# JakobHavtorn/benchmarking-lvms

Hardware: AMD Instinct MI355X
Metric: audio frames/sec training (VRNN, 16 kHz mu-law) (higher is better)
Workload: dtype f32

## Files before the change

### benchmarking-lvms_amd/csrc/pchain.h

```cpp
#pragma once
#include <algorithm>
#include <cstdlib>

#include "common.h"
#include "decode_tiles.h"

namespace blvm {
namespace pchain {

constexpr unsigned SENTINEL = 0xFFFFFFFFu;
constexpr unsigned SPIN_LIMIT = 1u << 22;

typedef unsigned u32x4 __attribute__((ext_vector_type(4)));
typedef __amdgpu_buffer_rsrc_t rsrc_t;
constexpr int AUX_SC1 = 16;
#ifndef PCHAIN_POLL_AUX
#define PCHAIN_POLL_AUX AUX_SC1
#endif
#ifndef PCHAIN_STORE_AUX
#define PCHAIN_STORE_AUX AUX_SC1
#endif
__device__ __forceinline__ rsrc_t make_rsrc(const void* base) {
  const unsigned long long u = reinterpret_cast<unsigned long long>(base);
  const unsigned lo = (unsigned)__builtin_amdgcn_readfirstlane((int)(unsigned)u), hi = (unsigned)__builtin_amdgcn_readfirstlane((int)(unsigned)(u >> 32));
// ... 1198 lines not shown
inline SeqLink rev_link(const float* W, const float* gate, float* orm, float* o16, long t0, long sB, int ld, long x16) {
  return SeqLink{W, gate ? gate + t0 * sB : nullptr, orm ? orm + t0 * sB : nullptr, -sB, ld, o16 ? o16 + t0 * x16 : nullptr};
}
inline int range_for(int tiles, int avail) { return std::max(8, std::min(avail & ~7, (tiles + 7) & ~7)); }

}

hipError_t pchain_fill_sentinel(void* p, size_t bytes, hipStream_t stream);
inline int pchain_ctl(pchain::Ctl& c) { return pchain_ctl(&c.dev, &c.host, &c.epoch); }
int pchain_prepare(pchain::Builder& bld, const char* who);
int pchain_run(const pchain::Program& prog, hipStream_t stream);
inline int pchain_launch(pchain::Builder& bld, const char* who, hipStream_t stream) {
  BLVM_TRY(pchain_prepare(bld, who));
  return pchain_run(bld.p, stream);
}
int vrnn_launch(pchain::Builder& bld, bool forward, const char* who, hipStream_t stream);
int pchain_rows_to_t16(const float* src, int ld, int B, int K, float* dst, hipStream_t stream, int n16 = 0, int k_src = 0);
struct StackPad {
  int S, Sp, N, Np;
  bool padded() const { return Sp != S; }
  size_t stage_in(int H) const { return padded() ? (size_t)H * Sp : 0; }
  size_t stage_dec(int H) const { return padded() ? (size_t)Np * H : 0; }
  size_t stage_bias() const { return padded() ? (size_t)Np : 0; }
};
inline StackPad stack_pad(int S, int F) {
  const int Sp = (S + 15) / 16 * 16, N = S * F;
  return StackPad{S, Sp, N, Sp != S ? (N + 15) / 16 * 16 : N};
}
inline int pad_copy(float* dst, int rows_p, int cols_p, const float* src, int rows, int cols, hipStream_t s) {
  BLVM_HIP(hipMemsetAsync(dst, 0, sizeof(float) * (size_t)rows_p * cols_p, s));
  BLVM_HIP(hipMemcpy2DAsync(dst, sizeof(float) * cols_p, src, sizeof(float) * cols, sizeof(float) * cols, rows, hipMemcpyDeviceToDevice, s));
// ... 21 lines not shown
```

### benchmarking-lvms_amd/csrc/vrnn.hip

```cpp
#include <vector>
#include <stdlib.h>

#include <algorithm>

#include "common.h"
#include "pchain.h"
#include "vrnn_static.h"

namespace blvm {
namespace {

#include "stages.h"


template <int NW>
__global__ __launch_bounds__(NW * 64) void gru_stage_kernel(const float* decin_t, const float* Wih, const float* xg,
                                                            const float* gh, int B, int H, int R, float* decin_next,
                                                            float* rg, float* ug, float* ng) {
  __shared__ float red[3 * NW * 256];
  const int r0 = blockIdx.y * 16, c0 = blockIdx.x * 16, wave = threadIdx.x >> 6;
  const int ldd = H + R;
  const int t = threadIdx.x & 255;
  const int row = r0 + (t >> 4), col = c0 + (t & 15);
  const bool own = threadIdx.x < 256 && row < B;
// ... 282 lines not shown
    BLVM_TRY(t16_pack_rows(w->post_w[l], H, H, H, rs.Wq[l], s));
  }
  BLVM_TRY(t16_pack_rows(w->prior_hw, H, 2 * Z, H, rs.Wph, s));
  BLVM_TRY(t16_pack_rows(w->post_hw, H, 2 * Z, H, rs.Wqh, s));
  BLVM_TRY(t16_pack_rows(w->phi_w[0], Z, H, Z, rs.Wf[0], s));
  for (int l = 1; l < 4; ++l) BLVM_TRY(t16_pack_rows(w->phi_w[l], H, H, H, rs.Wf[l], s));
  BLVM_TRY(t16_pack_rows(w->gru_wih + X, X + H, 3 * R, H, rs.Wih, s));
  BLVM_TRY(t16_pack_rows(w->gru_whh, R, 3 * R, R, rs.Whh, s));
  if (fold) {
    BLVM_TRY(t16_pack_rows(dec->w[0], H + R, H, H + R, rs.Wd[0], s));
    BLVM_TRY(t16_pack_rows(dec->w[1], H, H, H, rs.Wd[1], s));
    if (fold == 3) BLVM_TRY(t16_pack_rows(dec->w[2], H, SF, H, rs.Wd[2], s));
  }
  BLVM_TRY(pack_scope.flush());

  BLVM_HIP(copy_or_zero_2d(decin + H, sizeof(float) * ldd, h0, sizeof(float) * R, B, s));
  BLVM_HIP(hipMemset2DAsync(decin + n * ldd, sizeof(float) * ldd, 0, sizeof(float) * H, B, s));

  const int rt = (B + 15) / 16;
  if (vrnn_persistent(B) && device_cus() >= 32) {
    using namespace pchain;
    const int ctH = H / 16, ctZ = Z / 16, ctR = R / 16, cus = device_cus() & ~7;
    const long sH = (long)B * H, sZ = (long)B * Z, sR = (long)B * R, s3R = 3 * sR, sD = (long)B * ldd;
    const long xH = (long)rt * 16 * H, xZ = (long)rt * 16 * Z, xR = (long)rt * 16 * R;
    const bool groups = vrnn_row_groups(B);
    const int RTG = groups ? vrnn_rt(B) : 1;
    const int tl = (rt + RTG - 1) / RTG;
    const bool shared = vrnn_shared_deal(groups, tl);
    const VrnnFwdDeal dl = vrnn_fwd_deal(ctH, ctZ, ctR, tl, cus, shared, dec_ct(fold, SF));
    Builder bld;
    bld.begin(pchain_optype(B), Tp, B, groups ? 8 : 4, false, dl.g);
// ... 49 lines not shown
      o = Operands();
      o.p[LIN_A] = {rs.PHI16, xH}; o.p[LIN_W] = rs.Wd[0]; o.i[LIN_I_W_WIDTH] = ldw; o.p[LIN_ADD] = {rs.Y1P, sH}; o.ld[LIN_LD_ADD] = H;
      o.p[LIN_ORM] = {dec->y[0], sH}; o.ld[LD_OUT] = H; o.p[LIN_O16] = {rs.Y116, xH}; o.n16[N16_OUT] = ctH; o.f[LIN_F_SLOPE] = dec_slope;
      add_desc(bld, K_LIN, dl.dec[1].ct, dl.dec[1].wg0, dl.dec[1].nwg, H, DF_ADD_POLLED | DF_RELU | DF_GENTLE | canary, 0, Tp, o);
      o = Operands();
      o.p[LIN_A] = {rs.Y116, xH}; o.p[LIN_W] = rs.Wd[1]; o.p[LIN_BIAS] = dec->b[1]; o.p[LIN_ORM] = {dec->y[1], sH}; o.ld[LD_OUT] = H;
      o.p[LIN_O16] = {rs.Y216, xH}; o.n16[N16_OUT] = ctH; o.f[LIN_F_SLOPE] = dec_slope;
      add_desc(bld, K_LIN, dl.dec[2].ct, dl.dec[2].wg0, dl.dec[2].nwg, H, DF_RELU | DF_GENTLE | canary, 0, Tp, o);
      if (fold == 3) {
        o = Operands();
        o.p[LIN_A] = {rs.Y216, xH}; o.p[LIN_W] = rs.Wd[2]; o.p[LIN_BIAS] = dec->b[2]; o.p[LIN_ORM] = {dec->y[2], sF}; o.ld[LD_OUT] = SF;
        o.f[LIN_F_SLOPE] = dec_slope;
        add_desc(bld, K_LIN, dl.dec[3].ct, dl.dec[3].wg0, dl.dec[3].nwg, H, DF_RELU | DF_GENTLE | canary, 0, Tp, o);
      }
    }
    BLVM_HIP(pchain_fill_sentinel(rs.H16, rs.x16_bytes, s));
    BLVM_HIP(pchain_fill_sentinel(rs.GHb, sizeof(float) * n * 3 * R, s));
    BLVM_HIP(pchain_fill_sentinel(decin, sizeof(float) * n * ldd, s));
    BLVM_HIP(copy_or_zero_2d(decin + H, sizeof(float) * ldd, h0, sizeof(float) * R, B, s));
    BLVM_TRY(pchain_rows_to_t16(h0, R, B, R, rs.H16, s));
    BLVM_TRY(vrnn_launch(bld, true, "vrnn_fwd", s));
    if (fold) { ++g_dec_folded; if (folded) *folded = fold; }
    return BLVM_OK;
  }
  for (int t = 0; t < Tp; ++t) {
    const size_t oH = (size_t)t * B * H, oZ = (size_t)t * B * Z, oR = (size_t)t * B * R, o3R = (size_t)t * B * 3 * R;
    const float* dec_t = decin + (size_t)t * B * ldd;
    float* dec_n = decin + (size_t)(t + 1) * B * ldd;
    const float* hprev = dec_t + H;
    LinLaunch a;
    a.B = B;
    a.nseg = 3;
    a.seg[0] = seg(hprev, ldd, rs.Wp[0], R, w->prior_b[0], nullptr, 0, nullptr, 0, rs.P[0] + oH, H, H, R, 1);
    a.seg[1] = seg(hprev, ldd, rs.Wq[0], R, nullptr, rs.XQ + oH, H, nullptr, 0, rs.Q[0] + oH, H, H, R, 1);
    a.seg[2] = seg(hprev, ldd, rs.Whh, R, w->gru_bhh, nullptr, 0, nullptr, 0, rs.GHb + o3R, 3 * R, 3 * R, R, 0);
    launch_lin(a, s);
// ... 202 lines not shown
    {
      Operands z;
      z.p[DZ_D16] = last(ws.DPHI16[0], xH); z.p[DZ_WT] = ws.fT[0]; z.p[DZ_MU_Q] = last(mu_q, sZ); z.p[DZ_SD_Q] = last(sd_q, sZ); z.p[DZ_MU_P] = last(mu_p, sZ);
      z.p[DZ_SD_P] = last(sd_p, sZ); z.p[DZ_EPS] = last(eps, sZ); z.p[DZ_RAW_Q] = last(rs.RAWQ, sZ); z.p[DZ_RAW_P] = last(rs.RAWP, sZ); z.p[DZ_X_SL] = x_sl;
      z.p[DZ_C_RAW] = c_raw; z.p[DZ_C_FN] = c_fn; z.p[DZ_DQH] = last(ws.DQH, s2Z); z.p[DZ_DQH16] = last(ws.DQH16, x2Z); z.p[DZ_DPH] = last(ws.DPH, s2Z);
      z.p[DZ_DPH16] = last(ws.DPH16, x2Z); z.ld[LD_OUT] = 2 * Z; z.n16[N16_OUT] = 2 * ctZ; z.i[DZ_I_Z] = Z; z.i[DZ_I_RESIDUAL] = residual_posterior;
      z.i[DZ_I_STRIDE] = stride; z.i[DZ_I_T0] = T - 1; z.f[DZ_F_FN_FLOOR] = fn_floor; z.f[DZ_F_BETA] = beta; z.f[DZ_F_SD_EPS] = sd_eps;
      add_desc(bld, K_DZ, ctZ, dl.dz.wg0, dl.dz.nwg, H, 0, 0, T, z);
    }
    {
      const SeqLink lp[3] = {blink(ws.phT, rs.P[2], ws.DP[2], ws.DP16[2]), blink(ws.pT[2], rs.P[1], ws.DP[1], ws.DP16[1]), blink(ws.pT[1], rs.P[0], ws.DP[0], ws.DP16[0])};
      const SeqLink lq[3] = {blink(ws.qhT, rs.Q[2], ws.DQ[2], ws.DQ16[2]), blink(ws.qT[2], rs.Q[1], ws.DQ[1], ws.DQ16[1]), blink(ws.qT[1], rs.Q[0], ws.DQ[0], ws.DQ16[0])};
      add_linseq(bld, ctH, dl.prior.wg0, dl.prior.nwg, H, false, true, 0, T, last(ws.DPH16, x2Z), 3, lp, -sH, -xH, ctH, 0.f, H, 2 * Z);
      add_linseq(bld, ctH, dl.post.wg0, dl.post.nwg, H, false, true, 0, T, last(ws.DQH16, x2Z), 3, lq, -sH, -xH, ctH, 0.f, H, 2 * Z);
    }
    BLVM_HIP(pchain_fill_sentinel(ws.GA, ws.x16_bytes, s));
    BLVM_TRY(vrnn_launch(bld, false, "vrnn_bwd", s));
    if (split3) {
      const size_t n4 = n * H / 4;
      hipLaunchKernelGGL(add3_kernel, dim3((unsigned)std::min<size_t>((n4 + 255) / 256, 2048)), dim3(256), 0, s, reinterpret_cast<float4*>(ws.DPHI[3]),
                         reinterpret_cast<const float4*>(ws.DPHI3b), reinterpret_cast<const float4*>(ws.DPHI3c), n4);
    }
    return batched();
  }

  launch_dh(-1, Tp - 1);
  for (int t = Tp - 1; t >= 0; --t) {
    const size_t oH = (size_t)t * B * H, oZ = (size_t)t * B * Z, o3R = (size_t)t * B * 3 * R, o2Z = (size_t)t * B * 2 * Z;
    const float* dec_t = decin + (size_t)t * B * ldd;
    const float* ddec_t = d_decin + (size_t)t * B * ldd;
    LinLaunch a;
    a.B = B;
// ... 45 lines not shown
```

### benchmarking-lvms_amd/csrc/vrnn_static.h

```cpp
#pragma once
#include <algorithm>
#include <initializer_list>

#include "pchain.h"

namespace blvm {
namespace pchain {

struct LinkRange {
  int ct, wg0, nwg;
};
constexpr int kMaxTiles = 8;
struct VrnnFwdDeal {
  int def_n, half, g, spare;
  LinkRange hproj, prior, post, head, phi, gru, dec[4];
};
inline VrnnFwdDeal vrnn_fwd_deal(int ctH, int ctZ, int ctR, int tl, int cus, bool shared, int ctD = 0) {
  VrnnFwdDeal d;
  d.def_n = shared ? 0 : range_for(3 * ctR * tl, std::min(cus / 4, 64));
  d.half = range_for(ctH * tl, (cus - d.def_n) / 2);
  d.g = 2 * d.half;
  const int wide = shared ? d.half : d.g;
  d.hproj = shared ? LinkRange{3 * ctR, d.half, d.half} : LinkRange{3 * ctR, d.g, d.def_n};
  d.prior = LinkRange{ctH, 0, d.half};
// ... 68 lines not shown
    if (!kept) return false;
  }
  return true;
}
inline int place_for(int want, int fallback, const Program& p, int prior, int post, int grid) {
  if (want == kPlaceLocal) return place_local_applies(p, prior, post, grid) ? kPlaceLocal : (fallback == kPlacePlain ? kPlacePlain : kPlaceProgram);
  return want == kPlacePlain ? kPlacePlain : kPlaceProgram;
}
inline bool place_xcd(int place, const Program& p) { return place == kPlaceProgram && p.xcd != 0; }
inline int grid_of(const Program& p) {
  int g = 0;
  for (int i = 0; i < p.ndesc; ++i) g = std::max(g, p.d[i].wg0 + p.d[i].nwg);
  return g;
}

}
}
```

### benchmarking-lvms_amd/csrc/vrnn_static.hip

```cpp
#include <algorithm>
#include <mutex>

#include "common.h"
#include "pchain.h"
#include "vrnn_static.h"

namespace blvm {
namespace {
using namespace pchain;

struct SPtr {
  float* base;
  int stride;
  __device__ __forceinline__ float* at(int s) const { return base + (long)s * stride; }
};

__device__ __forceinline__ int placed_wg(int place) { return place == kPlaceLocal ? place_wg((int)blockIdx.x) : (int)blockIdx.x; }
__device__ __forceinline__ int tile_lanes(int w, int wg0, int nwg, int rt, int ct, bool xcd) {
  TileIter it(w, wg0, nwg, rt, ct, xcd);
  const int lane = threadIdx.x & 63;
  it.j += lane * it.step;
  return (lane < kMaxTiles && it.valid()) ? (it.r0() | (it.c() << 16)) : -1;
}
__device__ __forceinline__ int tile_count(int lanes) { return __popcll(__ballot(lanes >= 0)); }
// ... 281 lines not shown
  if (nt == 0 || s < d.s_begin || s >= d.s_end) return;
  wk.at(d, s, false);
  GrubIn g;
  g.D0 = q.D0.at(s); g.D1 = q.D1.at(s); g.W0 = q.W0; g.W1 = q.W1; g.g_in = q.g_in.at(s); g.g_add = q.g_add.at(s); g.ld_gadd = q.ld1;
  g.rg = q.rg.at(s); g.ug = q.ug.at(s); g.ng = q.ng.at(s); g.gh = q.gh.at(s); g.hprev = q.hprev.at(s); g.dd = q.dd.at(s); g.ldh = q.ld0;
  g.dgi = Out{q.dgi.at(s), q.ld3, false, q.dgi16.at(s), q.n16};
  g.dgh = Out{q.dgh.at(s), q.ld3, false, q.dgh16.at(s), q.n16};
  g.ga = q.ga.at(s); g.g_out = const_cast<float*>(q.g_out);
  g.has_gemm = s >= q.first_gemm; g.has_gates = s < q.end_gates; g.has_gin = s >= q.first_gin;
  const int trc = __builtin_amdgcn_readlane(tiles, 0);
  ANAT(anat_arm(wk.pl);)
  tile_grub<NW, OP_F32>(g, kH, q.R, trc & 0xffff, (trc >> 16) * 16, wk.B, wk.red(), wk.pl, ws, PC());
  ANAT(anat_note(wk.anat, 4 * d.idx, wk.pl);)
}

template <class A>
__device__ __forceinline__ const A& kargs() {
  typedef const __attribute__((address_space(4))) char kchar;
  kchar* p = (kchar*)__builtin_amdgcn_kernarg_segment_ptr();
  asm volatile("" : "+s"(p));
  return *(const A*)p;
}

struct FwdArgs {
  LinArgs hproj;
  SeqArgs run[2];
  HeadArgs head;
  SeqArgs phi;
  GruArgs gru;
  LinArgs dec[4];
  Deal deal[kFwdDecDesc];
  int ndec;
  int B, s0, S, xcd, place;
  Ctl ctl;
  ANAT(unsigned long long* prof;)
};
constexpr int kFwdProducts = 4, kBwdProducts = 2;

template <int NW, int HALF>
__device__ __forceinline__ void fwd_half(const FwdArgs& a, int w, int rt, bool xcd, Walk& wk) {
  const int t1 = tile_lanes(w, a.deal[1 + HALF].wg0, a.deal[1 + HALF].nwg, rt, a.deal[1 + HALF].ct, xcd), n1 = tile_count(t1);
  const int t3 = tile_lanes(w, a.deal[3].wg0, a.deal[3].nwg, rt, a.deal[3].ct, xcd), n3 = tile_count(t3);
  const int t4 = tile_lanes(w, a.deal[4].wg0, a.deal[4].nwg, rt, a.deal[4].ct, xcd), n4 = tile_count(t4);
  const int t5 = tile_lanes(w, a.deal[5].wg0, a.deal[5].nwg, rt, a.deal[5].ct, xcd), n5 = tile_count(t5);
  RunRes<3, kR, kH> run;
  Res<kH, 4> head;
  RunRes<4, kH, kH> phi;
  Res<kH, 3> gru;
  load_run<NW>(run, kargs<FwdArgs>().run[HALF], t1, n1);
  load_head<NW>(head, kargs<FwdArgs>().head, t3, n3);
  load_run<NW>(phi, kargs<FwdArgs>().phi, t4, n4);
  load_gru<NW>(gru, kargs<FwdArgs>().gru, t5, n5);
  for (int s = a.s0; s < a.S; ++s) {
    visit_run<NW, 3, kR, kH, false, Paced>(kargs<FwdArgs>().run[HALF], kargs<FwdArgs>().deal[1 + HALF], s, t1, n1, wk, run);
    visit_head<NW, Paced>(kargs<FwdArgs>().head, kargs<FwdArgs>().deal[3], s, t3, n3, wk, head);
    visit_run<NW, 4, kH, kH, false, Paced>(kargs<FwdArgs>().phi, kargs<FwdArgs>().deal[4], s, t4, n4, wk, phi);
    if constexpr (HALF == 0) visit_gru<NW, Paced>(kargs<FwdArgs>().gru, kargs<FwdArgs>().deal[5], s, t5, n5, wk, gru);
    else visit_gru<NW>(kargs<FwdArgs>().gru, kargs<FwdArgs>().deal[5], s, t5, n5, wk, gru);
  }
  ANAT(anat_end(wk.anat, kargs<FwdArgs>().prof, HALF, w == kargs<FwdArgs>().deal[1 + HALF].wg0);)
}

constexpr int kDecFlags = DF_RELU | DF_GENTLE | DF_CANARY;
template <int NW>
__device__ __forceinline__ void fwd_dec(const FwdArgs& a, int w, int rt, bool xcd, Walk& wk) {
  const int t6 = tile_lanes(w, a.deal[6].wg0, a.deal[6].nwg, rt, a.deal[6].ct, xcd), n6 = tile_count(t6);
  const int t7 = tile_lanes(w, a.deal[7].wg0, a.deal[7].nwg, rt, a.deal[7].ct, xcd), n7 = tile_count(t7);
  const int t8 = tile_lanes(w, a.deal[8].wg0, a.deal[8].nwg, rt, a.deal[8].ct, xcd), n8 = tile_count(t8);
  const int t9 = tile_lanes(w, a.deal[9].wg0, a.deal[9].nwg, rt, a.deal[9].ct, xcd), n9 = tile_count(t9);
  if ((n6 | n7 | n8 | n9) == 0) return;
  Res<kR> w1h;
  Res<kH> w1p, w2;
  load_lin<NW, kR>(w1h, kargs<FwdArgs>().dec[0].W, kargs<FwdArgs>().dec[0].w_width, t6, n6);
  load_lin<NW, kH>(w1p, kargs<FwdArgs>().dec[1].W, kargs<FwdArgs>().dec[1].w_width, t7, n7);
  load_lin<NW, kH>(w2, kargs<FwdArgs>().dec[2].W, kH, t8, n8);
  for (int s = a.s0; s < a.S; ++s) {
    visit_lin<NW, kR, DF_RM_SC1 | DF_GENTLE | DF_CANARY>(kargs<FwdArgs>().dec[0], kargs<FwdArgs>().deal[6], s, t6, n6, wk, w1h);
// ... 9 lines not shown
  const int w = placed_wg(a.place), rt = (a.B + 15) / 16;
  const bool xcd = a.place == kPlaceProgram && a.xcd != 0;
  Walk wk{lds_red, lds_red + kFwdProducts * NW * 256, 0, a.B, Poll{a.ctl, 0u, false, 1}};
  ANAT(__shared__ unsigned anat[kAnatSlots * 8]; anat_begin(anat); wk.anat = anat;)
  if (a.ndec != 0 && w >= a.deal[6].wg0) {
    fwd_dec<NW>(a, w, rt, xcd, wk);
    return;
  }
  if (w >= a.deal[0].wg0) {
    const int t0 = tile_lanes(w, a.deal[0].wg0, a.deal[0].nwg, rt, a.deal[0].ct, xcd), n0 = tile_count(t0);
    if (n0 == 0) return;
    for (int s = a.s0; s < a.S; ++s) visit_lin<NW, kR, DF_RM_SC1 | DF_GENTLE | DF_CANARY>(kargs<FwdArgs>().hproj, kargs<FwdArgs>().deal[0], s, t0, n0, wk, WMem());
    return;
  }
  if (w < a.deal[2].wg0) fwd_half<NW, 0>(a, w, rt, xcd, wk);
  else fwd_half<NW, 1>(a, w, rt, xcd, wk);
}

struct BwdArgs {
  GrubArgs grub;
  LinArgs part[3], gb, sum;
  SeqArgs phi;
  DzArgs dz;
  SeqArgs run[2];
  Deal deal[10];
  int B, s0, S, xcd, place;
  Ctl ctl;
  ANAT(unsigned long long* prof;)
};

template <int NW, int HALF>
__device__ __forceinline__ void bwd_half(const BwdArgs& a, int w, int rt, bool xcd, Walk& wk) {
  const int t0 = tile_lanes(w, a.deal[0].wg0, a.deal[0].nwg, rt, a.deal[0].ct, xcd), n0 = tile_count(t0);
  const int t1 = tile_lanes(w, a.deal[1 + HALF].wg0, a.deal[1 + HALF].nwg, rt, a.deal[1 + HALF].ct, xcd), n1 = tile_count(t1);
  const int t5 = tile_lanes(w, a.deal[5].wg0, a.deal[5].nwg, rt, a.deal[5].ct, xcd), n5 = tile_count(t5);
  const int t6 = tile_lanes(w, a.deal[6].wg0, a.deal[6].nwg, rt, a.deal[6].ct, xcd), n6 = tile_count(t6);
  const int t7 = tile_lanes(w, a.deal[7].wg0, a.deal[7].nwg, rt, a.deal[7].ct, xcd), n7 = tile_count(t7);
  const int t8 = tile_lanes(w, a.deal[8 + HALF].wg0, a.deal[8 + HALF].nwg, rt, a.deal[8 + HALF].ct, xcd), n8 = tile_count(t8);
  Res<kH, 2> grub;
  Res<kR> part;
  Res<kH> sum, dz;
  RunRes<2, kH, kH> phi;
// ... 16 lines not shown
  ANAT(anat_end(wk.anat, kargs<BwdArgs>().prof, 2 + HALF, w == kargs<BwdArgs>().deal[1 + HALF].wg0);)
}

template <int NW>
__global__ __launch_bounds__(NW * 64, 1) void vrnn_static_bwd_kernel(BwdArgs a) {
  extern __shared__ __attribute__((aligned(16))) float lds_red[];
  const int w = placed_wg(a.place), rt = (a.B + 15) / 16;
  const bool xcd = a.place == kPlaceProgram && a.xcd != 0;
  Walk wk{lds_red, lds_red + kBwdProducts * NW * 256, 0, a.B, Poll{a.ctl, 0u, false, 1}};
  ANAT(__shared__ unsigned anat[kAnatSlots * 8]; anat_begin(anat); wk.anat = anat;)
  if (w >= a.deal[3].wg0) {
    const int t = tile_lanes(w, a.deal[3].wg0, a.deal[3].nwg, rt, a.deal[3].ct, xcd), n = tile_count(t);
    if (n == 0) return;
    Res<kR> part;
    load_lin<NW, kR>(part, kargs<BwdArgs>().part[2].W, kargs<BwdArgs>().part[2].w_width, t, n);
    for (int s = a.s0; s < a.S; ++s) visit_lin<NW, kR, 0>(kargs<BwdArgs>().part[2], kargs<BwdArgs>().deal[3], s, t, n, wk, part);
    ANAT(anat_end(wk.anat, kargs<BwdArgs>().prof, 4, w == kargs<BwdArgs>().deal[3].wg0);)
    return;
  }
  if (w >= a.deal[4].wg0) {
    const int t = tile_lanes(w, a.deal[4].wg0, a.deal[4].nwg, rt, a.deal[4].ct, xcd), n = tile_count(t);
    if (n == 0) return;
    for (int s = a.s0; s < a.S; ++s)
      visit_lin<NW, 3 * kR, DF_ADD_POLLED | DF_RM_SC1 | DF_GENTLE | DF_CANARY>(kargs<BwdArgs>().gb, kargs<BwdArgs>().deal[4], s, t, n, wk, WMem());
    return;
  }
  if (w < a.deal[2].wg0) bwd_half<NW, 0>(a, w, rt, xcd, wk);
  else bwd_half<NW, 1>(a, w, rt, xcd, wk);
}

int static_place_fallback() { return (pchain_tune() & 32) ? kPlacePlain : kPlaceProgram; }
// ... 41 lines not shown
  ANAT(a.prof = pchain_profile_buffer();)
  const int grid = place == kPlaceLocal ? kPlaceSpan : d.wg0 + d.nwg;
  auto go = [&](auto kernel) -> int {
    BLVM_TRY(static_go(kernel, 2, grid, 0, "static_lin_chain"));
    hipLaunchKernelGGL(kernel, dim3(grid), dim3(1024), 0, stream, a);
    BLVM_CHECK_LAUNCH("static_lin_chain");
    return BLVM_OK;
  };
  if (resident && pace) return d.K == 256 ? go(&static_lin_chain_kernel<16, 256, true, PaceRt>) : go(&static_lin_chain_kernel<16, 512, true, PaceRt>);
  if (resident) return d.K == 256 ? go(&static_lin_chain_kernel<16, 256, true>) : go(&static_lin_chain_kernel<16, 512, true>);
  return d.K == 256 ? go(&static_lin_chain_kernel<16, 256, false>) : go(&static_lin_chain_kernel<16, 512, false>);
}

int g_static = 1;
long g_static_launches = 0;
bool pchain_static_on() { return g_static != 0; }

SPtr sp(const Program& p, const Desc& d, int k) { return SPtr{const_cast<float*>(d.p[k]), d.p[k] ? (int)p.stride[d.sidx[k]] : 0}; }
Deal deal_of(const Desc& d, int idx) { return Deal{d.wg0, d.nwg, d.ct, d.s_begin, d.s_end, idx}; }
bool within(const Desc& d, int lo, int hi) { return d.wg0 >= lo && d.wg0 + d.nwg <= hi; }
bool few_tiles(const Program& p, const Desc& d, bool xcd) {
  if (d.nwg <= 0 || (p.xcd && d.nwg % 8 != 0)) return false;
  return tiles_per_workgroup((p.B + 15) / 16, d.ct, d.nwg, xcd) <= kMaxTiles;
}
bool shaped(const Desc& d, int kind, int flags, int K) { return d.kind == kind && d.flags == flags && d.K == K; }
bool run(const Desc& d, int n, int K0) { return d.i[LINSEQ_I_N] == n && d.i[LINSEQ_I_K0] == K0; }

LinArgs lin_args(const Program& p, const Desc& d) {
  return LinArgs{sp(p, d, LIN_A), sp(p, d, LIN_A2), sp(p, d, LIN_A3), sp(p, d, LIN_ADD), sp(p, d, LIN_GATE), sp(p, d, LIN_ORM), sp(p, d, LIN_O16),
                 sp(p, d, LIN_O16B), d.p[LIN_W], d.p[LIN_BIAS], d.ld[LIN_LD_A], d.ld[LIN_LD_ADD], d.ld[LIN_LD_GATE], d.ld[LD_OUT], d.n16[N16_OUT], d.n16[N16_OUTB],
                 d.i[LIN_I_W_WIDTH], d.f[LIN_F_SLOPE]};
}
SeqArgs seq_args(const Program& p, const Desc& d) {
  SeqArgs q{};
  q.a0 = sp(p, d, LINSEQ_A0); q.add0 = sp(p, d, LINSEQ_ADD0);
  for (int i = 0; i < d.i[LINSEQ_I_N]; ++i) {
    q.W[i] = d.p[LINSEQ_W + i]; q.aux[i] = sp(p, d, LINSEQ_AUX + i); q.orm[i] = sp(p, d, LINSEQ_ORM + i); q.o16[i] = sp(p, d, LINSEQ_O16 + i);
    q.ld[i] = d.ld[LINSEQ_LD_ORM + i];
  }
  q.ldadd0 = d.i[LINSEQ_I_LD_ADD0]; q.ldgate = d.i[LINSEQ_I_LD_GATE]; q.n16 = d.n16[N16_OUT]; q.slope = d.f[LINSEQ_F_SLOPE];
  return q;
}

int vrnn_static_check(const Program& p, int ndesc, int products, int prior, int post, int* place) {
  if (!pchain_static_on() || p.ndesc != ndesc || p.ot != OP_F32 || p.rt_group != 1 || p.s_first != 0 || p.B > 64) return 1;
  if (p.lds_products != products || !int_strides(p)) return 1;
  *place = place_for(static_place_wanted(), static_place_fallback(), p, prior, post, grid_of(p));
  for (int i = 0; i < p.ndesc; ++i)
    if (!few_tiles(p, p.d[i], place_xcd(*place, p))) return 1;
  return 0;
}

int vrnn_static_fwd(const Program& p, hipStream_t stream) {
  int place = kPlaceProgram;
  const bool dec = p.ndesc == kFwdDecDesc || p.ndesc == kFwdDecDesc - 1;
  if (vrnn_static_check(p, dec ? p.ndesc : kFwdDesc, kFwdProducts, 1, 2, &place)) return 1;
  const Desc* d = p.d;
  const int S = p.S;
  for (int i = 0; i < p.ndesc; ++i)
    if (d[i].s_begin != 0 || d[i].s_end != S) return 1;
  if (!shaped(d[0], K_LIN, DF_RM_SC1 | DF_GENTLE | DF_CANARY, kR) || !shaped(d[1], K_LINSEQ, DF_RELU, kH) || !shaped(d[2], K_LINSEQ, DF_RELU, kH) ||
      !shaped(d[3], K_HEAD, 0, kH) || !shaped(d[4], K_LINSEQ, DF_RELU, kH) || !shaped(d[5], K_GRU, 0, kH))
    return 1;
  if (!run(d[1], 3, kR) || !run(d[2], 3, kR) || !run(d[4], 4, 0)) return 1;
  if (!one_tile_each(p, kFwdResident, place_xcd(place, p))) return 1;
  const int half = d[2].wg0, gentle = d[0].wg0;
  if (d[1].wg0 != 0 || !within(d[1], 0, half) || !within(d[2], half, gentle) || d[0].nwg <= 0) return 1;
  if (dec && !within(d[0], gentle, d[6].wg0)) return 1;
// ... 15 lines not shown
  a.run[0] = seq_args(p, d[1]); a.run[1] = seq_args(p, d[2]); a.phi = seq_args(p, d[4]);
  const Desc &h = d[3], &g = d[5];
  a.head = HeadArgs{sp(p, h, HEAD_P16), sp(p, h, HEAD_Q16), sp(p, h, HEAD_EPS), sp(p, h, HEAD_MU_P), sp(p, h, HEAD_SD_P), sp(p, h, HEAD_MU_Q),
                    sp(p, h, HEAD_SD_Q), sp(p, h, HEAD_RAW_P), sp(p, h, HEAD_RAW_Q), sp(p, h, HEAD_MUQ_RAW), sp(p, h, HEAD_Z), sp(p, h, HEAD_Z16),
                    sp(p, h, HEAD_Z16B), h.p[HEAD_WP], h.p[HEAD_BP], h.p[HEAD_WQ], h.p[HEAD_BQ], h.ld[LD_OUT], h.n16[N16_OUT], h.n16[N16_OUTB],
                    h.i[HEAD_I_Z], h.i[HEAD_I_RESIDUAL], h.f[HEAD_F_BETA], h.f[HEAD_F_INV_BETA], h.f[HEAD_F_SD_EPS]};
  a.gru = GruArgs{sp(p, g, GRU_X16), sp(p, g, GRU_XG), sp(p, g, GRU_GH), sp(p, g, GRU_HPREV), sp(p, g, GRU_HRM), sp(p, g, GRU_H16), sp(p, g, GRU_H16B),
                  sp(p, g, GRU_RG), sp(p, g, GRU_UG), sp(p, g, GRU_NG), g.p[GRU_WIH], g.p[GRU_BIH], g.ld[GRU_LD_HPREV], g.ld[LD_OUT], g.n16[N16_OUT],
                  g.n16[N16_OUTB], g.i[GRU_I_R]};
  a.ndec = dec ? p.ndesc - kFwdDesc : 0;
  for (int k = 0; k < a.ndec; ++k) a.dec[k] = lin_args(p, d[6 + k]);
  int grid = 0;
  for (int i = 0; i < p.ndesc; ++i) { a.deal[i] = deal_of(d[i], i); grid = std::max(grid, d[i].wg0 + d[i].nwg); }
  a.B = p.B; a.s0 = p.s_first; a.S = S; a.xcd = p.xcd; a.place = place; a.ctl = p.ctl;
  ANAT(a.prof = pchain_profile_buffer();)
  const size_t lds = sizeof(float) * 2 * kFwdProducts * 16 * 256;
  BLVM_TRY(static_go(&vrnn_static_fwd_kernel<16>, 0, grid, lds, "vrnn_static_fwd"));
  hipLaunchKernelGGL(vrnn_static_fwd_kernel<16>, dim3(grid), dim3(1024), lds, stream, a);
  BLVM_CHECK_LAUNCH("vrnn_static_fwd");
  ++g_static_launches;
  return BLVM_OK;
}

int vrnn_static_bwd(const Program& p, hipStream_t stream) {
  int place = kPlaceProgram;
  if (vrnn_static_check(p, 10, kBwdProducts, 8, 9, &place)) return 1;
  const Desc* d = p.d;
  const int S = p.S;
  for (int i = 0; i < 10; ++i)
    if (d[i].s_begin != 0 || d[i].s_end != (i == 0 ? S : S - 1)) return 1;
  if (!shaped(d[0], K_GRUB, 0, kH) || !shaped(d[1], K_LIN, 0, kR) || !shaped(d[2], K_LIN, 0, kR) || !shaped(d[3], K_LIN, 0, kR) ||
      !shaped(d[4], K_LIN, DF_ADD_POLLED | DF_RM_SC1 | DF_GENTLE | DF_CANARY, 3 * kR) || !shaped(d[5], K_LIN, DF_A_SUM3, kH) ||
      !shaped(d[6], K_LINSEQ, DF_SEQ_GATE, kH) || !shaped(d[7], K_DZ, 0, kH) || !shaped(d[8], K_LINSEQ, DF_SEQ_GATE, kH) ||
      !shaped(d[9], K_LINSEQ, DF_SEQ_GATE, kH))
    return 1;
  if (!run(d[6], 2, 0) || !run(d[8], 3, 2 * kH) || !run(d[9], 3, 2 * kH)) return 1;
  if (!one_tile_each(p, kBwdResident, place_xcd(place, p)) || d[7].p[DZ_D2_16] != nullptr) return 1;
  const int half = d[2].wg0, gentle = d[4].wg0, spare = d[3].wg0;
  if (!within(d[1], 0, half) || !within(d[8], 0, half) || !within(d[2], half, gentle) || !within(d[9], half, gentle) || !within(d[4], gentle, spare) ||
// ... 8 lines not shown
                    sp(p, g, GRUB_G_ADD), g.p[GRUB_W0], g.p[GRUB_W1], g.p[GRUB_G_OUT], g.ld[GRUB_LD_H], g.ld[GRUB_LD_GADD], g.ld[LD_OUT], g.n16[N16_OUT],
                    g.i[GRUB_I_R], g.i[GRUB_I_GEMM_FROM], g.i[GRUB_I_GATES_TO], g.i[GRUB_I_GIN_FROM]};
  for (int k = 0; k < 3; ++k) a.part[k] = lin_args(p, d[1 + k]);
  a.gb = lin_args(p, d[4]); a.sum = lin_args(p, d[5]);
  a.phi = seq_args(p, d[6]); a.run[0] = seq_args(p, d[8]); a.run[1] = seq_args(p, d[9]);
  const Desc& z = d[7];
  a.dz = DzArgs{sp(p, z, DZ_D16), sp(p, z, DZ_ADD), sp(p, z, DZ_MU_Q), sp(p, z, DZ_SD_Q), sp(p, z, DZ_MU_P), sp(p, z, DZ_SD_P),
                sp(p, z, DZ_EPS), sp(p, z, DZ_RAW_Q), sp(p, z, DZ_RAW_P), sp(p, z, DZ_MUQ_RAW), sp(p, z, DZ_DQH), sp(p, z, DZ_DQH16), sp(p, z, DZ_DPH),
                sp(p, z, DZ_DPH16), z.p[DZ_WT], z.p[DZ_C_RAW], z.p[DZ_C_FN], reinterpret_cast<const int32_t*>(z.p[DZ_X_SL]), z.ld[DZ_LD_ADD],
                z.ld[LD_OUT], z.n16[N16_OUT], z.i[DZ_I_Z], z.i[DZ_I_RESIDUAL], z.i[DZ_I_STRIDE], z.i[DZ_I_T0], (int)z.f[DZ_F_GEMM_FROM], z.f[DZ_F_FN_FLOOR],
                z.f[DZ_F_BETA], z.f[DZ_F_SD_EPS]};
  int grid = 0;
  for (int i = 0; i < 10; ++i) { a.deal[i] = deal_of(d[i], i); grid = std::max(grid, d[i].wg0 + d[i].nwg); }
  a.B = p.B; a.s0 = p.s_first; a.S = S; a.xcd = p.xcd; a.place = place; a.ctl = p.ctl;
  ANAT(a.prof = pchain_profile_buffer();)
  const size_t lds = sizeof(float) * 2 * kBwdProducts * 16 * 256;
  BLVM_TRY(static_go(&vrnn_static_bwd_kernel<16>, 1, grid, lds, "vrnn_static_bwd"));
  hipLaunchKernelGGL(vrnn_static_bwd_kernel<16>, dim3(grid), dim3(1024), lds, stream, a);
  BLVM_CHECK_LAUNCH("vrnn_static_bwd");
  ++g_static_launches;
  return BLVM_OK;
}

}

int vrnn_launch(pchain::Builder& bld, bool forward, const char* who, hipStream_t stream) {
  BLVM_TRY(pchain_prepare(bld, who));
  const int rc = forward ? vrnn_static_fwd(bld.p, stream) : vrnn_static_bwd(bld.p, stream);
  return rc == 1 ? pchain_run(bld.p, stream) : rc;
}

}

extern "C" int blvm_pchain_static(int mode) {
  if (mode == -2) return (int)std::min<long>(blvm::g_static_launches, 0x7fffffffL);
  const int was = blvm::g_static;
  if (mode >= 0) blvm::g_static = mode != 0;
  return was;
}

static int static_chain_probe(const float* W16, const float* bias, float* x16, float* xs, int B, int N, int L, int nwg, void* stream_, bool resident,
                              bool pace = false, int early = 0, int epi = 0) {
  using namespace blvm;
  using namespace blvm::pchain;
  hipStream_t s = static_cast<hipStream_t>(stream_);
  BLVM_REQUIRE(W16 && bias && x16 && xs && B > 0 && N > 0 && N % 16 == 0 && L > 0, "pchain_static_chain_probe: bad arguments");
  const int rt = (B + 15) / 16;
  const long x = (long)rt * 16 * N, sN = (long)B * N;
  Builder bld;
  bld.begin(OP_F32, L, B, 1, false, 0);
// ... 24 lines not shown
```

Baseline: 89.66 million.

## Replace full sentinel fills with in-kernel rolling arming of flag buffers

Instead of filling whole handshake buffers with sentinel values via separate memset-like launches before each persistent forward/backward kernel, a small prefix kernel arms only the first few timestep slabs. Idle or lightly loaded workgroups inside the persistent kernel then write sentinels a few steps ahead while the chain runs. This removes large pre-launch fill traffic from the critical path. In exchange it adds eligibility checks, extra stores inside the recurrent loop and ordering risk if arming races consumers, and it keeps the full-fill fallback when conditions are not met.

Result: faster. 91.28 million, median of 6 (+1.8%).

```diff
diff --git a/benchmarking-lvms_amd/csrc/pchain.h b/benchmarking-lvms_amd/csrc/pchain.h
--- a/benchmarking-lvms_amd/csrc/pchain.h
+++ b/benchmarking-lvms_amd/csrc/pchain.h
@@ -1,6 +1,7 @@
 #pragma once
 #include <algorithm>
 #include <cstdlib>
+#include <functional>
 
 #include "common.h"
 #include "decode_tiles.h"
@@ -1236,7 +1237,8 @@
   BLVM_TRY(pchain_prepare(bld, who));
   return pchain_run(bld.p, stream);
 }
-int vrnn_launch(pchain::Builder& bld, bool forward, const char* who, hipStream_t stream);
+namespace pchain { struct ArmPlan; }
+int vrnn_launch(pchain::Builder& bld, bool forward, const char* who, hipStream_t stream, const pchain::ArmPlan& plan, const std::function<int()>& pre);
 int pchain_rows_to_t16(const float* src, int ld, int B, int K, float* dst, hipStream_t stream, int n16 = 0, int k_src = 0);
 struct StackPad {
   int S, Sp, N, Np;
diff --git a/benchmarking-lvms_amd/csrc/vrnn.hip b/benchmarking-lvms_amd/csrc/vrnn.hip
--- a/benchmarking-lvms_amd/csrc/vrnn.hip
+++ b/benchmarking-lvms_amd/csrc/vrnn.hip
@@ -320,7 +320,7 @@
   }
   BLVM_TRY(pack_scope.flush());
 
-  BLVM_HIP(copy_or_zero_2d(decin + H, sizeof(float) * ldd, h0, sizeof(float) * R, B, s));
+  if (!(vrnn_persistent(B) && device_cus() >= 32)) BLVM_HIP(copy_or_zero_2d(decin + H, sizeof(float) * ldd, h0, sizeof(float) * R, B, s));
   BLVM_HIP(hipMemset2DAsync(decin + n * ldd, sizeof(float) * ldd, 0, sizeof(float) * H, B, s));
 
   const int rt = (B + 15) / 16;
@@ -400,12 +400,25 @@
         add_desc(bld, K_LIN, dl.dec[3].ct, dl.dec[3].wg0, dl.dec[3].nwg, H, DF_RELU | DF_GENTLE | canary, 0, Tp, o);
       }
     }
-    BLVM_HIP(pchain_fill_sentinel(rs.H16, rs.x16_bytes, s));
-    BLVM_HIP(pchain_fill_sentinel(rs.GHb, sizeof(float) * n * 3 * R, s));
-    BLVM_HIP(pchain_fill_sentinel(decin, sizeof(float) * n * ldd, s));
-    BLVM_HIP(copy_or_zero_2d(decin + H, sizeof(float) * ldd, h0, sizeof(float) * R, B, s));
-    BLVM_TRY(pchain_rows_to_t16(h0, R, B, R, rs.H16, s));
-    BLVM_TRY(vrnn_launch(bld, true, "vrnn_fwd", s));
+    ArmPlan plan;
+    plan.fill(rs.H16, rs.x16_bytes);
+    plan.fill(rs.GHb, sizeof(float) * n * 3 * R);
+    plan.fill(decin, sizeof(float) * n * ldd);
+    if (!groups) {
+      plan.add(arm_t16(rs.H16, R, rt, Tp + 1));
+      for (int i = 0; i < 3; ++i) { plan.add(arm_t16(rs.P16[i], H, rt, Tp)); plan.add(arm_t16(rs.Q16[i], H, rt, Tp)); plan.add(arm_t16(rs.FZ16[i], H, rt, Tp)); }
+      plan.add(arm_t16(rs.Z16, Z, rt, Tp));
+      plan.add(arm_t16(rs.PHI16, H, rt, Tp));
+      plan.add(arm_t16(rs.Y116, H, rt, Tp)); plan.add(arm_t16(rs.Y216, H, rt, Tp));
+      plan.add(arm_rm(rs.Y1P, H, B, Tp));
+      plan.add(arm_rm(rs.GHb, 3 * R, B, Tp));
+      plan.add(arm_rm(decin, ldd, B, Tp));
+    }
+    auto pre = [&]() -> int {
+      BLVM_HIP(copy_or_zero_2d(decin + H, sizeof(float) * ldd, h0, sizeof(float) * R, B, s));
+      return pchain_rows_to_t16(h0, R, B, R, rs.H16, s);
+    };
+    BLVM_TRY(vrnn_launch(bld, true, "vrnn_fwd", s, plan, pre));
     if (fold) { ++g_dec_folded; if (folded) *folded = fold; }
     return BLVM_OK;
   }
@@ -638,8 +651,17 @@
       add_linseq(bld, ctH, dl.prior.wg0, dl.prior.nwg, H, false, true, 0, T, last(ws.DPH16, x2Z), 3, lp, -sH, -xH, ctH, 0.f, H, 2 * Z);
       add_linseq(bld, ctH, dl.post.wg0, dl.post.nwg, H, false, true, 0, T, last(ws.DQH16, x2Z), 3, lq, -sH, -xH, ctH, 0.f, H, 2 * Z);
     }
-    BLVM_HIP(pchain_fill_sentinel(ws.GA, ws.x16_bytes, s));
-    BLVM_TRY(vrnn_launch(bld, false, "vrnn_bwd", s));
+    ArmPlan plan;
+    plan.fill(ws.GA, ws.x16_bytes);
+    if (!groups) {
+      plan.add(arm_rm(ws.GA, R, B, T, true)); plan.add(arm_rm(ws.GB, R, B, T, true));
+      for (int i = 0; i < 3; ++i) { plan.add(arm_t16(ws.DP16[i], H, rt, T, true)); plan.add(arm_t16(ws.DQ16[i], H, rt, T, true)); }
+      plan.add(arm_t16(ws.DGI16, 3 * R, rt, T, true)); plan.add(arm_t16(ws.DGH16, 3 * R, rt, T, true));
+      for (int i = 0; i < 4; ++i) plan.add(arm_t16(ws.DPHI16[i], H, rt, T, true));
+      plan.add(arm_t16(ws.DPH16, 2 * Z, rt, T, true)); plan.add(arm_t16(ws.DQH16, 2 * Z, rt, T, true));
+      plan.add(arm_t16(ws.DPHI16b, H, rt, T, true)); plan.add(arm_t16(ws.DPHI16c, H, rt, T, true));
+    }
+    BLVM_TRY(vrnn_launch(bld, false, "vrnn_bwd", s, plan, []() -> int { return BLVM_OK; }));
     if (split3) {
       const size_t n4 = n * H / 4;
       hipLaunchKernelGGL(add3_kernel, dim3((unsigned)std::min<size_t>((n4 + 255) / 256, 2048)), dim3(256), 0, s, reinterpret_cast<float4*>(ws.DPHI[3]),
diff --git a/benchmarking-lvms_amd/csrc/vrnn_static.h b/benchmarking-lvms_amd/csrc/vrnn_static.h
--- a/benchmarking-lvms_amd/csrc/vrnn_static.h
+++ b/benchmarking-lvms_amd/csrc/vrnn_static.h
@@ -106,5 +106,100 @@
   return g;
 }
 
-}
-}
+constexpr int kArmAhead = 4;
+constexpr int kArmMax = 24;
+constexpr int kArmCandidates = 64;
+struct ArmEntry {
+  float* base;
+  int step, tile, n4, n4_last, nslabs;
+};
+struct ArmTable {
+  ArmEntry e[kArmMax];
+  int n;
+};
+inline ArmEntry arm_t16(float* buf, int width, int rt, int nslabs, bool reversed = false) {
+  const int step = rt * 16 * width;
+  return ArmEntry{reversed ? buf + (long)(nslabs - 1) * step : buf, reversed ? -step : step, 16 * width, 4 * width, 4 * width, nslabs};
+}
+inline ArmEntry arm_rm(float* buf, int ld, int B, int nslabs, bool reversed = false) {
+  const int step = B * ld, rt = (B + 15) / 16;
+  return ArmEntry{reversed ? buf + (long)(nslabs - 1) * step : buf, reversed ? -step : step, 16 * ld, 4 * ld, (B - 16 * (rt - 1)) * ld / 4, nslabs};
+}
+struct ArmPlan {
+  ArmTable tab{};
+  struct Region { void* p; size_t bytes; } full[3] = {};
+  int nfull = 0;
+  void add(const ArmEntry& e) { if (e.base != nullptr && tab.n < kArmMax) tab.e[tab.n++] = e; else if (e.base != nullptr) tab.n = kArmMax + 1; }
+  void fill(void* p, size_t bytes) { full[nfull++] = Region{p, bytes}; }
+};
+__host__ __device__ __forceinline__ void arm_share(const ArmEntry& e, int r, int rt, int k, int log2n, int* first, int* count) {
+  const int total = r == rt - 1 ? e.n4_last : e.n4, per = (total + (1 << log2n) - 1) >> log2n;
+  *first = k * per < total ? k * per : total;
+  *count = per < total - *first ? per : total - *first;
+}
+inline bool arm_rank(const Program& p, int link, int cand0, int ncand, bool xcd, int w, int* r, int* k, int* n) {
+  const int rt = (p.B + 15) / 16;
+  const Desc& d = p.d[link];
+  TileIter mine(w, d.wg0, d.nwg, rt, d.ct, xcd);
+  if (w < cand0 || w >= cand0 + ncand || !mine.valid()) return false;
+  *r = mine.r0() / 16; *k = 0; *n = 0;
+  for (int c = cand0; c < cand0 + ncand; ++c) {
+    TileIter it(c, d.wg0, d.nwg, rt, d.ct, xcd);
+    if (!it.valid() || it.r0() != mine.r0()) continue;
+    ++*n;
+    if (c < w) ++*k;
+  }
+  return true;
+}
+inline int arm_operand_slot(int kind) {
+  switch (kind) {
+    case K_LIN: return LIN_A;
+    case K_LINSEQ: return LINSEQ_A0;
+    case K_HEAD: return HEAD_P16;
+    case K_GRU: return GRU_X16;
+    case K_GRUB: return GRUB_D0_16;
+    case K_DZ: return DZ_D16;
+    default: return -1;
+  }
+}
+inline bool arm_applies(const Program& p, const ArmTable& t, int link, std::initializer_list<int> idle, int cand0, int ncand, bool xcd) {
+  const int rt = (p.B + 15) / 16;
+  if (t.n <= 0 || t.n > kArmMax || ncand <= 0 || ncand > kArmCandidates || p.S <= kArmAhead || p.rt_group != 1) return false;
+  for (int i = 0; i < t.n; ++i) {
+    const ArmEntry& e = t.e[i];
+    const long span = e.step < 0 ? -(long)e.step : e.step;
+    if (e.base == nullptr || (reinterpret_cast<unsigned long long>(e.base) & 15) != 0 || e.step % 4 != 0 || e.tile % 4 != 0) return false;
+    if (e.n4 <= 0 || e.n4_last <= 0 || e.n4_last > e.n4 || 4L * e.n4 > e.tile || (long)(rt - 1) * e.tile + 4L * e.n4_last > span) return false;
+    if (e.nslabs < p.S - 1 || e.nslabs > p.S + 1) return false;
+  }
+  for (int i = 0; i < p.ndesc; ++i) {
+    const Desc& d = p.d[i];
+    const int slot = arm_operand_slot(d.kind);
+    if (slot < 0 || d.p[slot] == nullptr || p.stride[d.sidx[slot]] == 0) return false;
+    bool inside = false;
+    for (int k = 0; k < t.n && !inside; ++k) {
+      const ArmEntry& e = t.e[k];
+      const long span = e.step < 0 ? -(long)e.step : e.step;
+      const float* lo = e.step < 0 ? e.base - (long)(e.nslabs - 1) * span : e.base;
+      inside = d.p[slot] >= lo && d.p[slot] <= lo + (long)e.nslabs * span;
+    }
+    if (!inside) return false;
+  }
+  const Desc& d = p.d[link];
+  int armers[4] = {0, 0, 0, 0};
+  if (rt > 4) return false;
+  for (int w = cand0; w < cand0 + ncand; ++w) {
+    int tiles = 0, r = 0;
+    for (TileIter it(w, d.wg0, d.nwg, rt, d.ct, xcd); it.valid(); it.next()) { ++tiles; r = it.r0() / 16; }
+    if (tiles > 1) return false;
+    if (tiles == 1) ++armers[r];
+    for (int i : idle)
+      if (TileIter(w, p.d[i].wg0, p.d[i].nwg, rt, p.d[i].ct, xcd).valid()) return false;
+  }
+  for (int r = 0; r < rt; ++r)
+    if (armers[r] == 0 || (armers[r] & (armers[r] - 1)) != 0) return false;
+  return true;
+}
+
+}
+}
diff --git a/benchmarking-lvms_amd/csrc/vrnn_static.hip b/benchmarking-lvms_amd/csrc/vrnn_static.hip
--- a/benchmarking-lvms_amd/csrc/vrnn_static.hip
+++ b/benchmarking-lvms_amd/csrc/vrnn_static.hip
@@ -319,6 +319,33 @@
   ANAT(anat_note(wk.anat, 4 * d.idx, wk.pl);)
 }
 
+struct Armer {
+  int r, k, log2n;
+};
+__device__ __forceinline__ Armer arm_rank_dev(int w, const Deal& link, int cand0, int ncand, int rt, bool xcd, int tiles, int nt, int entries) {
+  if (entries == 0 || nt != 1 || w < cand0 || w >= cand0 + ncand) return Armer{0, 0, -1};
+  const int lane = threadIdx.x & 63, my_r0 = __builtin_amdgcn_readlane(tiles, 0) & 0xffff;
+  const TileIter it(cand0 + lane, link.wg0, link.nwg, rt, link.ct, xcd);
+  const unsigned long long same = __ballot(lane < ncand && it.valid() && it.r0() == my_r0);
+  const int n = (int)__popcll(same);
+  return Armer{my_r0 >> 4, (int)__popcll(same & ((1ull << (w - cand0)) - 1ull)), __builtin_ctz((unsigned)n)};
+}
+template <int NW>
+__device__ __forceinline__ void arm_ahead(const ArmTable& t, int j, int rt, const Armer& a) {
+  if (a.log2n < 0) return;
+  const int lane = threadIdx.x & 63, wave = __builtin_amdgcn_readfirstlane((int)(threadIdx.x >> 6));
+  const u32x4 ff = {SENTINEL, SENTINEL, SENTINEL, SENTINEL};
+  for (int e = wave; e < t.n; e += NW) {
+    const ArmEntry& en = t.e[e];
+    if (j >= en.nslabs) continue;
+    int first, count;
+    arm_share(en, a.r, rt, a.k, a.log2n, &first, &count);
+    const rsrc_t dst = make_rsrc(en.base + (long)j * en.step + (long)a.r * en.tile + 4L * first);
+    for (int i = lane; i < count; i += 64) __builtin_amdgcn_raw_buffer_store_b128(ff, dst, 16 * i, 0, PCHAIN_STORE_AUX);
+  }
+  asm volatile("s_waitcnt vmcnt(0)" ::: "memory");
+}
+
 template <class A>
 __device__ __forceinline__ const A& kargs() {
   typedef const __attribute__((address_space(4))) char kchar;
@@ -338,6 +365,7 @@
   int ndec;
   int B, s0, S, xcd, place;
   Ctl ctl;
+  ArmTable arm;
   ANAT(unsigned long long* prof;)
 };
 constexpr int kFwdProducts = 4, kBwdProducts = 2;
@@ -366,6 +394,23 @@
   ANAT(anat_end(wk.anat, kargs<FwdArgs>().prof, HALF, w == kargs<FwdArgs>().deal[1 + HALF].wg0);)
 }
 
+template <int NW>
+__device__ __forceinline__ void fwd_post_arming(const FwdArgs& a, int w, int rt, bool xcd, Walk& wk) {
+  const int t1 = tile_lanes(w, a.deal[2].wg0, a.deal[2].nwg, rt, a.deal[2].ct, xcd), n1 = tile_count(t1);
+  const int t5 = tile_lanes(w, a.deal[5].wg0, a.deal[5].nwg, rt, a.deal[5].ct, xcd), n5 = tile_count(t5);
+  const Armer armer = arm_rank_dev(w, a.deal[5], a.deal[2].wg0, a.deal[0].wg0 - a.deal[2].wg0, rt, xcd, t5, n5, a.arm.n);
+  RunRes<3, kR, kH> run;
+  Res<kH, 3> gru;
+  load_run<NW>(run, kargs<FwdArgs>().run[1], t1, n1);
+  load_gru<NW>(gru, kargs<FwdArgs>().gru, t5, n5);
+  for (int s = a.s0; s < a.S; ++s) {
+    visit_run<NW, 3, kR, kH, false, Paced>(kargs<FwdArgs>().run[1], kargs<FwdArgs>().deal[2], s, t1, n1, wk, run);
+    arm_ahead<NW>(kargs<FwdArgs>().arm, s + kArmAhead, rt, armer);
+    visit_gru<NW>(kargs<FwdArgs>().gru, kargs<FwdArgs>().deal[5], s, t5, n5, wk, gru);
+  }
+  ANAT(anat_end(wk.anat, kargs<FwdArgs>().prof, 1, w == kargs<FwdArgs>().deal[2].wg0);)
+}
+
 constexpr int kDecFlags = DF_RELU | DF_GENTLE | DF_CANARY;
 template <int NW>
 __device__ __forceinline__ void fwd_dec(const FwdArgs& a, int w, int rt, bool xcd, Walk& wk) {
@@ -405,6 +450,7 @@
     return;
   }
   if (w < a.deal[2].wg0) fwd_half<NW, 0>(a, w, rt, xcd, wk);
+  else if (a.arm.n != 0) fwd_post_arming<NW>(a, w, rt, xcd, wk);
   else fwd_half<NW, 1>(a, w, rt, xcd, wk);
 }
 
@@ -417,6 +463,7 @@
   Deal deal[10];
   int B, s0, S, xcd, place;
   Ctl ctl;
+  ArmTable arm;
   ANAT(unsigned long long* prof;)
 };
 
@@ -463,7 +510,11 @@
     if (n == 0) return;
     Res<kR> part;
     load_lin<NW, kR>(part, kargs<BwdArgs>().part[2].W, kargs<BwdArgs>().part[2].w_width, t, n);
-    for (int s = a.s0; s < a.S; ++s) visit_lin<NW, kR, 0>(kargs<BwdArgs>().part[2], kargs<BwdArgs>().deal[3], s, t, n, wk, part);
+    const Armer armer = arm_rank_dev(w, a.deal[3], a.deal[3].wg0, a.deal[3].nwg, rt, xcd, t, n, a.arm.n);
+    for (int s = a.s0; s < a.S; ++s) {
+      visit_lin<NW, kR, 0>(kargs<BwdArgs>().part[2], kargs<BwdArgs>().deal[3], s, t, n, wk, part);
+      arm_ahead<NW>(kargs<BwdArgs>().arm, s + kArmAhead, rt, armer);
+    }
     ANAT(anat_end(wk.anat, kargs<BwdArgs>().prof, 4, w == kargs<BwdArgs>().deal[3].wg0);)
     return;
   }
@@ -535,6 +586,7 @@
 
 int g_static = 1;
 long g_static_launches = 0;
+long g_armed_launches = 0;
 bool pchain_static_on() { return g_static != 0; }
 
 SPtr sp(const Program& p, const Desc& d, int k) { return SPtr{const_cast<float*>(d.p[k]), d.p[k] ? (int)p.stride[d.sidx[k]] : 0}; }
@@ -561,6 +613,31 @@
   }
   q.ldadd0 = d.i[LINSEQ_I_LD_ADD0]; q.ldgate = d.i[LINSEQ_I_LD_GATE]; q.n16 = d.n16[N16_OUT]; q.slope = d.f[LINSEQ_F_SLOPE];
   return q;
+}
+
+__global__ __launch_bounds__(256) void arm_prefix_kernel(ArmTable t, int rt) {
+  const ArmEntry& en = t.e[blockIdx.y];
+  const uint4 ff = make_uint4(SENTINEL, SENTINEL, SENTINEL, SENTINEL);
+  const int slabs = en.nslabs < kArmAhead ? en.nslabs : kArmAhead;
+  for (int j = 0; j < slabs; ++j)
+    for (int r = 0; r < rt; ++r) {
+      uint4* const dst = reinterpret_cast<uint4*>(en.base + (long)j * en.step + (long)r * en.tile);
+      const int n4 = r == rt - 1 ? en.n4_last : en.n4;
+      for (int i = blockIdx.x * 256 + threadIdx.x; i < n4; i += gridDim.x * 256) dst[i] = ff;
+    }
+}
+int full_fill(const ArmPlan& plan, hipStream_t stream) {
+  for (int i = 0; i < plan.nfull; ++i) BLVM_HIP(pchain_fill_sentinel(plan.full[i].p, plan.full[i].bytes, stream));
+  return BLVM_OK;
+}
+int arm_or_fill(const Program& p, const ArmPlan& plan, int link, std::initializer_list<int> idle, int cand0, int ncand, bool xcd, hipStream_t stream,
+                ArmTable* arm) {
+  arm->n = 0;
+  if ((pchain_tune() & 128) != 0 || !arm_applies(p, plan.tab, link, idle, cand0, ncand, xcd)) return full_fill(plan, stream);
+  *arm = plan.tab;
+  hipLaunchKernelGGL(arm_prefix_kernel, dim3(8, plan.tab.n), dim3(256), 0, stream, plan.tab, (p.B + 15) / 16);
+  BLVM_CHECK_LAUNCH("arm_prefix");
+  return BLVM_OK;
 }
 
 int vrnn_static_check(const Program& p, int ndesc, int products, int prior, int post, int* place) {
@@ -572,7 +649,7 @@
   return 0;
 }
 
-int vrnn_static_fwd(const Program& p, hipStream_t stream) {
+int vrnn_static_fwd(const Program& p, hipStream_t stream, const ArmPlan& plan, const std::function<int()>& pre) {
   int place = kPlaceProgram;
   const bool dec = p.ndesc == kFwdDecDesc || p.ndesc == kFwdDecDesc - 1;
   if (vrnn_static_check(p, dec ? p.ndesc : kFwdDesc, kFwdProducts, 1, 2, &place)) return 1;
@@ -618,15 +695,18 @@
   for (int i = 0; i < p.ndesc; ++i) { a.deal[i] = deal_of(d[i], i); grid = std::max(grid, d[i].wg0 + d[i].nwg); }
   a.B = p.B; a.s0 = p.s_first; a.S = S; a.xcd = p.xcd; a.place = place; a.ctl = p.ctl;
   ANAT(a.prof = pchain_profile_buffer();)
+  BLVM_TRY(arm_or_fill(p, plan, 5, {3, 4}, half, gentle - half, place_xcd(place, p), stream, &a.arm));
+  BLVM_TRY(pre());
   const size_t lds = sizeof(float) * 2 * kFwdProducts * 16 * 256;
   BLVM_TRY(static_go(&vrnn_static_fwd_kernel<16>, 0, grid, lds, "vrnn_static_fwd"));
   hipLaunchKernelGGL(vrnn_static_fwd_kernel<16>, dim3(grid), dim3(1024), lds, stream, a);
   BLVM_CHECK_LAUNCH("vrnn_static_fwd");
   ++g_static_launches;
+  if (a.arm.n != 0) ++g_armed_launches;
   return BLVM_OK;
 }
 
-int vrnn_static_bwd(const Program& p, hipStream_t stream) {
+int vrnn_static_bwd(const Program& p, hipStream_t stream, const ArmPlan& plan, const std::function<int()>& pre) {
   int place = kPlaceProgram;
   if (vrnn_static_check(p, 10, kBwdProducts, 8, 9, &place)) return 1;
   const Desc* d = p.d;
@@ -665,26 +745,33 @@
   for (int i = 0; i < 10; ++i) { a.deal[i] = deal_of(d[i], i); grid = std::max(grid, d[i].wg0 + d[i].nwg); }
   a.B = p.B; a.s0 = p.s_first; a.S = S; a.xcd = p.xcd; a.place = place; a.ctl = p.ctl;
   ANAT(a.prof = pchain_profile_buffer();)
+  BLVM_TRY(arm_or_fill(p, plan, 3, {}, spare, d[3].nwg, place_xcd(place, p), stream, &a.arm));
+  BLVM_TRY(pre());
   const size_t lds = sizeof(float) * 2 * kBwdProducts * 16 * 256;
   BLVM_TRY(static_go(&vrnn_static_bwd_kernel<16>, 1, grid, lds, "vrnn_static_bwd"));
   hipLaunchKernelGGL(vrnn_static_bwd_kernel<16>, dim3(grid), dim3(1024), lds, stream, a);
   BLVM_CHECK_LAUNCH("vrnn_static_bwd");
   ++g_static_launches;
+  if (a.arm.n != 0) ++g_armed_launches;
   return BLVM_OK;
 }
 
 }
 
-int vrnn_launch(pchain::Builder& bld, bool forward, const char* who, hipStream_t stream) {
+int vrnn_launch(pchain::Builder& bld, bool forward, const char* who, hipStream_t stream, const pchain::ArmPlan& plan, const std::function<int()>& pre) {
   BLVM_TRY(pchain_prepare(bld, who));
-  const int rc = forward ? vrnn_static_fwd(bld.p, stream) : vrnn_static_bwd(bld.p, stream);
-  return rc == 1 ? pchain_run(bld.p, stream) : rc;
+  const int rc = forward ? vrnn_static_fwd(bld.p, stream, plan, pre) : vrnn_static_bwd(bld.p, stream, plan, pre);
+  if (rc != 1) return rc;
+  BLVM_TRY(full_fill(plan, stream));
+  BLVM_TRY(pre());
+  return pchain_run(bld.p, stream);
 }
 
 }
 
 extern "C" int blvm_pchain_static(int mode) {
   if (mode == -2) return (int)std::min<long>(blvm::g_static_launches, 0x7fffffffL);
+  if (mode == -3) return (int)std::min<long>(blvm::g_armed_launches, 0x7fffffffL);
   const int was = blvm::g_static;
   if (mode >= 0) blvm::g_static = mode != 0;
   return was;
```
